# selftok-team/SelftokTokenizer

Hardware: NVIDIA H100
Metric: images/sec encode+50-step decode, 256x256/512-tok (higher is better)
Workload: dtype fp16 (IEEE-half operands on wgmma, fp32 accumulate; encoder/VQ/tables fp32)

## Files before the change

### selftoktokenizer_b200/csrc/gemm_tc.cu

```cuda
#include "common.cuh"
#include "hopper.cuh"
#include "kernels.h"

#include <stdlib.h>

namespace stk {

namespace {

using namespace hop;

constexpr int BM = 128, BN = 256, BK = 64, WK = 16;
constexpr int A_TILE_BYTES = BM * BK * 2;
constexpr int B_TILE_BYTES = BN * BK * 2;
constexpr int CONSUMERS = 2;
constexpr int NUM_THREADS = CONSUMERS * 128 + 128;
constexpr int PRODUCER_REGS = 40, CONSUMER_REGS = 232;
constexpr int ACC = BN / 2;
constexpr int kPrefetchKBlocks = 4;

template <int NSPLIT> struct Cfg {
  static constexpr int PLANES = NSPLIT == 3 ? 2 : 1;
  static constexpr int STAGE_BYTES = PLANES * (A_TILE_BYTES + B_TILE_BYTES);
  static constexpr int STAGES = NSPLIT == 3 ? 2 : 4;
  static constexpr int SMEM_BYTES = STAGES * STAGE_BYTES + 1024  + 256 ;
};

__device__ __forceinline__ void wgmma_tile(float (&d)[ACC], uint64_t da, uint64_t db, uint32_t acc, bool fp16) {
  if (fp16) wgmma_m64n256k16_ss_f16(d, da, db, acc);
  else wgmma_m64n256k16_ss_bf16(d, da, db, acc);
}

__device__ __forceinline__ float2 ldg2(const float* p) { return *reinterpret_cast<const float2*>(p); }

struct EpiRows {
  int orow[2], mrow[2];
  bool valid[2];
};

__device__ __forceinline__ EpiRows epilogue_rows(const Epilogue& e, int64_t row0, int64_t M) {
  const bool per_row_gate = e.mode == EPI_RESID && e.gate && (e.gate_period > 1 || e.tab_rows);
  const bool per_row_add = e.mode == EPI_STORE && e.addtab;
  EpiRows rw;
#pragma unroll
  for (int r = 0; r < 2; ++r) {
    const int64_t m = row0 + 8 * r;
    rw.valid[r] = m < M;
    const int mi = (int)m;
    rw.orow[r] = 0;
    if (e.row_map && rw.valid[r]) {
      rw.orow[r] = e.row_map[mi];
    } else if (e.plan && rw.valid[r]) {
      const int b = mi / e.rpb_in;
      const int n_img = e.rpb_out - (e.plan_ctx ? e.rpb_in : e.row_off);
      rw.orow[r] = b * e.rpb_out + plan_slot_row(mi % e.rpb_in, e.plan[2 * b], e.plan[2 * b + 1], n_img, e.plan_ctx != 0);
    } else if (rw.valid[r]) {
      rw.orow[r] = e.rpb_in > 0 ? (mi / e.rpb_in) * e.rpb_out + e.row_off + (mi % e.rpb_in) : mi;
    }
    if (e.tab_rows && rw.valid[r]) rw.mrow[r] = e.tab_rows[mi];
    else rw.mrow[r] = per_row_gate ? mi % e.gate_period : (per_row_add ? mi % e.add_period : 0);
  }
  return rw;
}

__device__ __forceinline__ void epilogue_prefetch(const Epilogue& e, const EpiRows& rw, int col0, int N) {
  if (e.mode != EPI_RESID) return;
  const int c0 = col0 & ~(BN - 1);
  const int q = (col0 >> 1) & 3;
#pragma unroll
  for (int r = 0; r < 2; ++r) {
#pragma unroll
    for (int h = 0; h < 2; ++h) {
      const int n = c0 + 32 * (2 * q + h);
      if (rw.valid[r] && n < N) prefetch_l2(e.resid + (int64_t)rw.orow[r] * e.ldo + n);
    }
  }
}

template <int MODE, bool GELU>
__device__ __forceinline__ void epilogue_tile(const Epilogue& e, const float (&acc)[ACC], const EpiRows& rw, int col0, int N) {
  constexpr int CH = MODE == EPI_RESID ? 4 : 8;
  const bool per_row_gate = MODE == EPI_RESID && e.gate && (e.gate_period > 1 || e.tab_rows);
  const bool per_row_add = MODE == EPI_STORE && e.addtab;
  const bool fp16 = e.fp16 != 0;
  const float2 zero = make_float2(0.f, 0.f), one = make_float2(1.f, 1.f);
#pragma unroll
  for (int c = 0; c < BN / 8; c += CH) {
    float2 bias[CH], res[2][CH], gt[2][CH], add[2][CH];
#pragma unroll
    for (int i = 0; i < CH; ++i) {
      const int n = col0 + 8 * (c + i);
      const bool in = n < N;
      bias[i] = e.bias && in ? ldg2(e.bias + n) : zero;
#pragma unroll
      for (int r = 0; r < 2; ++r) {
        const bool v = in && rw.valid[r];
        const int64_t o = (int64_t)rw.orow[r] * e.ldo + n;
        if (MODE == EPI_RESID) {
          res[r][i] = v ? ldg2(e.resid + o) : zero;
          gt[r][i] = v && e.gate ? ldg2(per_row_gate ? e.gate + (int64_t)rw.mrow[r] * e.gate_ld + n : e.gate + n) : one;
        }
        if (MODE == EPI_STORE) add[r][i] = v && per_row_add ? ldg2(e.addtab + (int64_t)rw.mrow[r] * e.add_ld + n) : zero;
      }
    }
#pragma unroll
    for (int i = 0; i < CH; ++i) {
      const int j = c + i;
      const int n = col0 + 8 * j;
      if (n >= N) continue;
#pragma unroll
      for (int r = 0; r < 2; ++r) {
        if (!rw.valid[r]) continue;
        float2 y = make_float2(acc[4 * j + 2 * r] + bias[i].x, acc[4 * j + 2 * r + 1] + bias[i].y);
        if (GELU) y = gelu_tanh_fast2(y);
        const int64_t o = (int64_t)rw.orow[r] * e.ldo + n;
        if (MODE == EPI_RESID) {
          y.x = fmaf(gt[r][i].x, y.x, res[r][i].x); y.y = fmaf(gt[r][i].y, y.y, res[r][i].y);
        }
        if (MODE == EPI_SPLIT) {
          const uint32_t hi = pack2_sat16(y.x, y.y, fp16);
          *reinterpret_cast<uint32_t*>(e.out_hi + o) = hi;
          if (e.out_lo) {
            const float lx = y.x - __bfloat162float(__float2bfloat16_rn(y.x)), ly = y.y - __bfloat162float(__float2bfloat16_rn(y.y));
            *reinterpret_cast<uint32_t*>(e.out_lo + o) = pack2_sat16(lx, ly, false);
          }
        } else {
          if (per_row_add) { y.x += add[r][i].x; y.y += add[r][i].y; }
          *reinterpret_cast<float2*>(e.out + o) = y;
        }
      }
    }
  }
}

__device__ __forceinline__ void epilogue_dispatch(const Epilogue& e, const float (&acc)[ACC], const EpiRows& rw, int col0, int N) {
  if (e.mode == EPI_RESID) epilogue_tile<EPI_RESID, false>(e, acc, rw, col0, N);
  else if (e.mode == EPI_SPLIT) {
    if (e.act == ACT_GELU) epilogue_tile<EPI_SPLIT, true>(e, acc, rw, col0, N);
    else epilogue_tile<EPI_SPLIT, false>(e, acc, rw, col0, N);
  } else {
    if (e.act == ACT_GELU) epilogue_tile<EPI_STORE, true>(e, acc, rw, col0, N);
    else epilogue_tile<EPI_STORE, false>(e, acc, rw, col0, N);
  }
}

struct TcMaps {
  CUtensorMap a_hi, a_lo, b_hi, b_lo;
};

struct GemmParams {
  int64_t M;
  int N, K;
  int fp16;
  Epilogue ep;
  int conv_C = 0, conv_H = 0, conv_W = 0, conv_stride = 1;
  int raster_gm = 4;
};

__device__ __forceinline__ void tile_coords(int t, int pm_tiles, int n_tiles, int GM, int& pm, int& n_blk) {
  const int per_group = GM * n_tiles;
  const int group = t / per_group;
  const int first = group * GM;
  const int gm = min(GM, pm_tiles - first);
  const int local = t - group * per_group;
  pm = first + local % gm;
  n_blk = local / gm;
}

template <int NSPLIT, int CL, bool FP16>
__global__ void __launch_bounds__(NUM_THREADS, 1)
gemm_tc_kernel(const __grid_constant__ TcMaps maps0, const __grid_constant__ TcMaps maps1, const GemmParams p0, const GemmParams p1) {
  static_assert(NSPLIT == 1 || !FP16, "the fp16 mode is single-pass");
  using C = Cfg<NSPLIT>;
  extern __shared__ uint8_t smem_raw[];
  const uint32_t smem_base = (smem_u32(smem_raw) + 1023u) & ~1023u;
  const uint32_t bar_base = smem_base + C::STAGES * C::STAGE_BYTES;
  auto full_bar = [&](int s) { return bar_base + 8u * s; };
  auto empty_bar = [&](int s) { return bar_base + 8u * (C::STAGES + s); };

  const int warp = threadIdx.x >> 5, lane = threadIdx.x & 31;
  const uint32_t rank = CL > 1 ? cluster_ctarank() : 0;
  const int pm_tiles0 = (int)((p0.M + CL * BM - 1) / (CL * BM)), n_tiles0 = (p0.N + BN - 1) / BN;
  const int pm_tiles1 = (int)((p1.M + CL * BM - 1) / (CL * BM)), n_tiles1 = (p1.N + BN - 1) / BN;
  const int tiles0 = pm_tiles0 * n_tiles0;
  const int num_tiles = tiles0 + pm_tiles1 * n_tiles1;
  const int cluster_id = blockIdx.x / CL, num_clusters = gridDim.x / CL;

  if (warp == CONSUMERS * 4 && lane == 0) {
    tma_prefetch_desc(&maps0.a_hi);
    tma_prefetch_desc(&maps0.b_hi);
    if (NSPLIT == 3) { tma_prefetch_desc(&maps0.a_lo); tma_prefetch_desc(&maps0.b_lo); }
    if (p1.M > 0) {
      tma_prefetch_desc(&maps1.a_hi);
      tma_prefetch_desc(&maps1.b_hi);
      if (NSPLIT == 3) { tma_prefetch_desc(&maps1.a_lo); tma_prefetch_desc(&maps1.b_lo); }
    }
    for (int s = 0; s < C::STAGES; ++s) { mbar_init(full_bar(s), 1); mbar_init(empty_bar(s), CONSUMERS * CL); }
    asm volatile("fence.mbarrier_init.release.cluster;" ::: "memory");
  }
  __syncthreads();
  if (CL > 1) cluster_sync_all();

  if (warp >= CONSUMERS * 4) {
    setmaxnreg_dec<PRODUCER_REGS>();
    if (warp == CONSUMERS * 4 && lane == 0) {
      int stage = 0; uint32_t phase = 0;
      const uint64_t w_policy = l2_policy_evict_last();
      for (int t = cluster_id; t < num_tiles; t += num_clusters) {
        const bool second = t >= tiles0;
        const TcMaps& mp = second ? maps1 : maps0;
        const GemmParams& pp = second ? p1 : p0;
        int pm, n_blk;
        if (second) tile_coords(t - tiles0, pm_tiles1, n_tiles1, p1.raster_gm, pm, n_blk);
        else tile_coords(t, pm_tiles0, n_tiles0, p0.raster_gm, pm, n_blk);
        const int nk = (pp.K + BK - 1) / BK;
        const int m_row = (pm * CL + (int)rank) * BM;
        const int n_row = n_blk * BN + (int)rank * (BN / CL);
        const int chunks = pp.conv_C > 0 ? pp.conv_C / BK : 1;
        int cx = 0, cy = 0, cb = 0;
        if (pp.conv_C > 0) {
          cx = m_row % pp.conv_W;
          cy = (m_row / pp.conv_W) % pp.conv_H;
          cb = m_row / (pp.conv_W * pp.conv_H);
        }
        for (int kb = 0; kb < nk; ++kb) {
          mbar_wait(empty_bar(stage), phase ^ 1);
          const uint32_t sa = smem_base + stage * C::STAGE_BYTES;
          const uint32_t sb = sa + C::PLANES * A_TILE_BYTES + (uint32_t)rank * (B_TILE_BYTES / CL);
          const uint32_t fb = full_bar(stage);
          mbar_expect_tx(fb, C::STAGE_BYTES);
          if (pp.conv_C > 0) {
            const int tap = kb / chunks, c0 = (kb - tap * chunks) * BK;
            const int dy = tap / 3, dx = tap - dy * 3;
            int x0 = cx + dx - 1, y0 = cy + dy - 1, n0 = cb;
            if (pp.conv_stride == 2) { x0 = cx + (dx >> 1); y0 = cy + (dy >> 1); n0 = cb * 4 + (dy & 1) * 2 + (dx & 1); }
            tma_load_4d(sa, &mp.a_hi, fb, c0, x0, y0, n0);
            if (NSPLIT == 3) tma_load_4d(sa + A_TILE_BYTES, &mp.a_lo, fb, c0, x0, y0, n0);
          } else {
            tma_load_2d(sa, &mp.a_hi, fb, kb * BK, m_row);
            if (NSPLIT == 3) tma_load_2d(sa + A_TILE_BYTES, &mp.a_lo, fb, kb * BK, m_row);
          }
          if (CL > 1) {
            tma_load_2d_mc(sb, &mp.b_hi, fb, kb * BK, n_row, (uint16_t)((1u << CL) - 1), w_policy);
            if (NSPLIT == 3) tma_load_2d_mc(sb + B_TILE_BYTES, &mp.b_lo, fb, kb * BK, n_row, (uint16_t)((1u << CL) - 1), w_policy);
          } else {
            tma_load_2d_hint(sb, &mp.b_hi, fb, kb * BK, n_row, w_policy);
            if (NSPLIT == 3) tma_load_2d_hint(sb + B_TILE_BYTES, &mp.b_lo, fb, kb * BK, n_row, w_policy);
          }
          if (++stage == C::STAGES) { stage = 0; phase ^= 1; }
        }
      }
    }
  } else {
    setmaxnreg_inc<CONSUMER_REGS>();
    const int wg = warp >> 2;
    const bool signaller = (threadIdx.x & 127) == 0;
    auto release = [&](int s) {
      if (!signaller) return;
      if (CL == 1) mbar_arrive(empty_bar(s));
      else for (int r = 0; r < CL; ++r) mbar_arrive_cluster(empty_bar(s), (uint32_t)r);
    };
    int stage = 0; uint32_t phase = 0;
    for (int t = cluster_id; t < num_tiles; t += num_clusters) {
      const bool second = t >= tiles0;
      int pm, n_blk;
      if (second) tile_coords(t - tiles0, pm_tiles1, n_tiles1, p1.raster_gm, pm, n_blk);
      else tile_coords(t, pm_tiles0, n_tiles0, p0.raster_gm, pm, n_blk);
      const int nk = ((second ? p1.K : p0.K) + BK - 1) / BK;
      const int wl = threadIdx.x & 127;
      const int64_t row0 = (int64_t)(pm * CL + (int)rank) * BM + wg * 64 + (wl >> 5) * 16 + ((wl & 31) >> 2);
      const int col0 = n_blk * BN + 2 * (wl & 3);
      const EpiRows rw = second ? epilogue_rows(p1.ep, row0, p1.M) : epilogue_rows(p0.ep, row0, p0.M);
      const int pf_kb = nk > kPrefetchKBlocks ? nk - kPrefetchKBlocks : 0;
      float acc[ACC];
#pragma unroll
      for (int i = 0; i < ACC; ++i) acc[i] = 0.f;
      int prev = -1;
      for (int kb = 0; kb < nk; ++kb) {
        mbar_wait(full_bar(stage), phase);
        const uint32_t sa_hi = smem_base + stage * C::STAGE_BYTES + wg * (64 * 128);
        const uint32_t sa_lo = sa_hi + A_TILE_BYTES;
        const uint32_t sb_hi = smem_base + stage * C::STAGE_BYTES + C::PLANES * A_TILE_BYTES;
        const uint32_t sb_lo = sb_hi + B_TILE_BYTES;
        wgmma_fence();
#pragma unroll
        for (int k = 0; k < BK / WK; ++k) {
          const uint32_t koff = k * WK * 2;
          const uint64_t da_hi = make_smem_desc(sa_hi + koff), db_hi = make_smem_desc(sb_hi + koff);
          wgmma_tile(acc, da_hi, db_hi, (kb > 0 || k > 0) ? 1u : 0u, FP16);
          if (NSPLIT == 3) {
            const uint64_t da_lo = make_smem_desc(sa_lo + koff), db_lo = make_smem_desc(sb_lo + koff);
            wgmma_tile(acc, da_hi, db_lo, 1u, false);
            wgmma_tile(acc, da_lo, db_hi, 1u, false);
          }
        }
        wgmma_commit();
        if (kb == pf_kb) {
          if (!second) epilogue_prefetch(p0.ep, rw, col0, p0.N);
          else epilogue_prefetch(p1.ep, rw, col0, p1.N);
        }
        wgmma_wait<1>();
        if (prev >= 0) release(prev);
        prev = stage;
        if (++stage == C::STAGES) { stage = 0; phase ^= 1; }
      }
      wgmma_wait<0>();
      fence_regs(acc);
      release(prev);
      if (!second) epilogue_dispatch(p0.ep, acc, rw, col0, p0.N);
      else epilogue_dispatch(p1.ep, acc, rw, col0, p1.N);
    }
  }
  if (CL > 1) cluster_sync_all();
}

typedef CUresult (*EncodeTiledFn)(CUtensorMap*, CUtensorMapDataType, cuuint32_t, void*, const cuuint64_t*, const cuuint64_t*,
                                  const cuuint32_t*, const cuuint32_t*, CUtensorMapInterleave, CUtensorMapSwizzle,
                                  CUtensorMapL2promotion, CUtensorMapFloatOOBfill);
EncodeTiledFn g_encode = nullptr;
constexpr int kMaxDev = 64;
int g_num_sms_dev[kMaxDev];
bool g_attr_dev[kMaxDev];
int g_raster_gm = 4;
int g_gemm_ctas = 2;

int make_map(CUtensorMap* map, const __nv_bfloat16* ptr, int64_t rows, int K, int box_rows, int fp16) {
  cuuint64_t gdim[2] = {(cuuint64_t)K, (cuuint64_t)rows};
  cuuint64_t gstride[1] = {(cuuint64_t)K * 2};
  cuuint32_t box[2] = {(cuuint32_t)BK, (cuuint32_t)box_rows};
  cuuint32_t estr[2] = {1, 1};
  CUresult r = g_encode(map, fp16 ? CU_TENSOR_MAP_DATA_TYPE_FLOAT16 : CU_TENSOR_MAP_DATA_TYPE_BFLOAT16, 2, const_cast<__nv_bfloat16*>(ptr), gdim, gstride, box, estr,
                        CU_TENSOR_MAP_INTERLEAVE_NONE, CU_TENSOR_MAP_SWIZZLE_128B, CU_TENSOR_MAP_L2_PROMOTION_L2_256B,
                        CU_TENSOR_MAP_FLOAT_OOB_FILL_NONE);
  if (r != CUDA_SUCCESS) {
    set_error("cuTensorMapEncodeTiled failed with CUresult " + std::to_string((int)r));
    return -5;
  }
  return 0;
}

int make_map_nhwc(CUtensorMap* map, const __nv_bfloat16* ptr, int64_t B, int H, int W, int Cc, int fp16) {
  const int bw = W < BM ? W : BM;
  const int bh = (BM / bw) < H ? (BM / bw) : H;
  const int bn = BM / (bw * bh);
  cuuint64_t gdim[4] = {(cuuint64_t)Cc, (cuuint64_t)W, (cuuint64_t)H, (cuuint64_t)B};
  cuuint64_t gstride[3] = {(cuuint64_t)Cc * 2, (cuuint64_t)W * Cc * 2, (cuuint64_t)H * W * Cc * 2};
  cuuint32_t box[4] = {(cuuint32_t)BK, (cuuint32_t)bw, (cuuint32_t)bh, (cuuint32_t)bn};
  cuuint32_t estr[4] = {1, 1, 1, 1};
  CUresult r = g_encode(map, fp16 ? CU_TENSOR_MAP_DATA_TYPE_FLOAT16 : CU_TENSOR_MAP_DATA_TYPE_BFLOAT16, 4, const_cast<__nv_bfloat16*>(ptr), gdim, gstride,
                        box, estr, CU_TENSOR_MAP_INTERLEAVE_NONE, CU_TENSOR_MAP_SWIZZLE_128B, CU_TENSOR_MAP_L2_PROMOTION_L2_256B,
                        CU_TENSOR_MAP_FLOAT_OOB_FILL_NONE);
  if (r != CUDA_SUCCESS) {
    set_error("cuTensorMapEncodeTiled (NHWC) failed with CUresult " + std::to_string((int)r));
    return -5;
  }
  return 0;
}

}

int make_tensor_map_2d(CUtensorMap* map, const void* ptr, uint64_t rows, uint64_t cols, uint32_t box_rows, uint32_t box_cols,
                       int fp16) {
  STK_CHECK(g_encode, -3, "gemm_tc_init has not been called");
  cuuint64_t gdim[2] = {(cuuint64_t)cols, (cuuint64_t)rows};
  cuuint64_t gstride[1] = {(cuuint64_t)cols * 2};
  cuuint32_t box[2] = {box_cols, box_rows};
  cuuint32_t estr[2] = {1, 1};
  CUresult r = g_encode(map, fp16 ? CU_TENSOR_MAP_DATA_TYPE_FLOAT16 : CU_TENSOR_MAP_DATA_TYPE_BFLOAT16, 2, const_cast<void*>(ptr), gdim,
                        gstride, box, estr, CU_TENSOR_MAP_INTERLEAVE_NONE, CU_TENSOR_MAP_SWIZZLE_128B,
                        CU_TENSOR_MAP_L2_PROMOTION_L2_256B, CU_TENSOR_MAP_FLOAT_OOB_FILL_NONE);
  if (r != CUDA_SUCCESS) {
    set_error("cuTensorMapEncodeTiled failed with CUresult " + std::to_string((int)r));
    return -5;
  }
  return 0;
}

void gemm_tc_set_ctas(int n) { g_gemm_ctas = n == 1 ? 1 : 2; }

int gemm_tc_init() {
  int dev = 0;
  STK_CUDA(cudaGetDevice(&dev));
  STK_CHECK(dev >= 0 && dev < kMaxDev, -1, "gemm_tc: device ordinal out of range");
  if (g_encode && g_attr_dev[dev]) return 0;
  if (!g_encode) {
    void* fn = nullptr;
    cudaDriverEntryPointQueryResult qres;
    STK_CUDA(cudaGetDriverEntryPoint("cuTensorMapEncodeTiled", &fn, cudaEnableDefault, &qres));
    STK_CHECK(fn && qres == cudaDriverEntryPointSuccess, -5, "cuTensorMapEncodeTiled not available from the driver");
    const char* v = getenv("SELFTOK_GEMM_CTAS");
    if (v) g_gemm_ctas = atoi(v) == 1 ? 1 : 2;
    const char* gm = getenv("SELFTOK_GEMM_GM");
    if (gm && atoi(gm) >= 1 && atoi(gm) <= 1024) g_raster_gm = atoi(gm);
    g_encode = reinterpret_cast<EncodeTiledFn>(fn);
  }
  STK_CUDA(cudaDeviceGetAttribute(&g_num_sms_dev[dev], cudaDevAttrMultiProcessorCount, dev));
  STK_CUDA(cudaFuncSetAttribute(gemm_tc_kernel<1, 1, false>, cudaFuncAttributeMaxDynamicSharedMemorySize, Cfg<1>::SMEM_BYTES));
  STK_CUDA(cudaFuncSetAttribute(gemm_tc_kernel<1, 1, true>, cudaFuncAttributeMaxDynamicSharedMemorySize, Cfg<1>::SMEM_BYTES));
  STK_CUDA(cudaFuncSetAttribute(gemm_tc_kernel<3, 1, false>, cudaFuncAttributeMaxDynamicSharedMemorySize, Cfg<3>::SMEM_BYTES));
  STK_CUDA(cudaFuncSetAttribute(gemm_tc_kernel<1, 2, false>, cudaFuncAttributeMaxDynamicSharedMemorySize, Cfg<1>::SMEM_BYTES));
  STK_CUDA(cudaFuncSetAttribute(gemm_tc_kernel<1, 2, true>, cudaFuncAttributeMaxDynamicSharedMemorySize, Cfg<1>::SMEM_BYTES));
  STK_CUDA(cudaFuncSetAttribute(gemm_tc_kernel<3, 2, false>, cudaFuncAttributeMaxDynamicSharedMemorySize, Cfg<3>::SMEM_BYTES));
  g_attr_dev[dev] = true;
  return 0;
}

int check_gemm_tc_problem(const TcProblem& q, int nsplit, int fp16) {
  const Epilogue& ep = q.ep;
  STK_CHECK(q.A_hi && q.W_hi && q.M > 0 && q.N > 0 && q.K > 0, -1, "gemm_tc: bad arguments");
  STK_CHECK(nsplit == 1 || (nsplit == 3 && q.A_lo && q.W_lo), -1, "gemm_tc: nsplit must be 1, or 3 with lo planes");
  STK_CHECK(!fp16 || nsplit == 1, -1, "gemm_tc: the fp16 mode is single-pass");
  auto aligned16 = [](const void* p) { return reinterpret_cast<uintptr_t>(p) % 16 == 0; };
  STK_CHECK(aligned16(q.A_hi) && aligned16(q.A_lo) && aligned16(q.W_hi) && aligned16(q.W_lo), -1,
            "gemm_tc: operand planes must be 16-byte aligned (TMA)");
  STK_TRY(check_epilogue(ep, "gemm_tc"));
  STK_CHECK(ep.act == ACT_NONE || (ep.act == ACT_GELU && ep.mode != EPI_RESID), -2,
            "gemm_tc: epilogue activation must be none, or GELU-tanh with the store / split modes");
  STK_CHECK(ep.mode != EPI_STORE || ep.addtab == nullptr || ep.add_ld % 4 == 0, -2, "gemm_tc: addtab pitch must be a multiple of 4");
  STK_CHECK(q.K % 8 == 0, -2, "gemm_tc: K must be a multiple of 8 (16-byte TMA row pitch)");
  STK_CHECK(ep.ldo % 4 == 0 && q.N % 4 == 0, -2, "gemm_tc: N and the output pitch must be multiples of 4");
  STK_CHECK(ep.mode != EPI_RESID || ep.gate == nullptr || ep.gate_ld % 4 == 0, -2, "gemm_tc: gate pitch must be a multiple of 4");
  if (q.conv_C > 0) {
    STK_CHECK(q.conv_C % BK == 0 && q.K == 9 * q.conv_C, -2, "gemm_tc conv: channels must be a multiple of 64 and K = 9 C");
    STK_CHECK(q.conv_W > 0 && q.conv_H > 0 && (q.conv_W % BM == 0 || BM % q.conv_W == 0), -2, "gemm_tc conv: image width must divide or be a multiple of 128");
    const int64_t hw = (int64_t)q.conv_H * q.conv_W;
    STK_CHECK(q.M % hw == 0 && (hw % BM == 0 || BM % hw == 0) && (q.conv_W >= BM || hw < BM || q.conv_H % (BM / q.conv_W) == 0), -2,
              "gemm_tc conv: 128-pixel tiles must be part of a row, whole rows of one image, or whole images");
    STK_CHECK(q.conv_stride == 1 || (q.conv_stride == 2 && hw % BM == 0), -2, "gemm_tc conv: stride 2 needs >= 128 output pixels per image");
  }
  return 0;
}

static int make_maps(TcMaps* m, const TcProblem& q, int nsplit, int fp16, int b_box) {
  const bool conv = q.conv_C > 0;
  const int64_t imgs = conv ? q.M / ((int64_t)q.conv_H * q.conv_W) * (q.conv_stride == 2 ? 4 : 1) : 0;
  if (conv) STK_TRY(make_map_nhwc(&m->a_hi, q.A_hi, imgs, q.conv_H, q.conv_W, q.conv_C, fp16));
  else STK_TRY(make_map(&m->a_hi, q.A_hi, q.M, q.K, BM, fp16));
  STK_TRY(make_map(&m->b_hi, q.W_hi, q.N, q.K, b_box, fp16));
  if (nsplit == 3) {
    if (conv) STK_TRY(make_map_nhwc(&m->a_lo, q.A_lo, imgs, q.conv_H, q.conv_W, q.conv_C, fp16));
    else STK_TRY(make_map(&m->a_lo, q.A_lo, q.M, q.K, BM, fp16));
    STK_TRY(make_map(&m->b_lo, q.W_lo, q.N, q.K, b_box, fp16));
  } else {
    m->a_lo = m->a_hi; m->b_lo = m->b_hi;
  }
  return 0;
}

template <int NSPLIT, int CL, bool FP16>
static int launch_kernel(const TcMaps& m0, const TcMaps& m1, const GemmParams& p0, const GemmParams& p1, int clusters, cudaStream_t s) {
  cudaLaunchConfig_t cfg = {};
  cfg.gridDim = dim3(CL * clusters);
  cfg.blockDim = dim3(NUM_THREADS);
  cfg.dynamicSmemBytes = Cfg<NSPLIT>::SMEM_BYTES;
  cfg.stream = s;
  cudaLaunchAttribute attr[1];
  attr[0].id = cudaLaunchAttributeClusterDimension;
  attr[0].val.clusterDim.x = CL; attr[0].val.clusterDim.y = 1; attr[0].val.clusterDim.z = 1;
  cfg.attrs = attr;
  cfg.numAttrs = 1;
  STK_CUDA(cudaLaunchKernelEx(&cfg, gemm_tc_kernel<NSPLIT, CL, FP16>, m0, m1, p0, p1));
  count_launch();
  return 0;
}

template <int CL>
static int launch_cl(const TcMaps& m0, const TcMaps& m1, const GemmParams& p0, const GemmParams& p1, int clusters, int nsplit, int fp16,
                     cudaStream_t s) {
  if (nsplit == 3) return launch_kernel<3, CL, false>(m0, m1, p0, p1, clusters, s);
  if (fp16) return launch_kernel<1, CL, true>(m0, m1, p0, p1, clusters, s);
  return launch_kernel<1, CL, false>(m0, m1, p0, p1, clusters, s);
}

int launch_gemm_tc_grouped(const TcProblem* probs, int n, int nsplit, cudaStream_t s, int fp16) {
  STK_TRY(gemm_tc_init());
  STK_CHECK(probs && (n == 1 || n == 2), -1, "gemm_tc: one or two problems per launch");
  int dev = 0;
  STK_CUDA(cudaGetDevice(&dev));
  const int g_num_sms = g_num_sms_dev[dev];
  for (int i = 0; i < n; ++i) STK_TRY(check_gemm_tc_problem(probs[i], nsplit, fp16));
  const int CL = g_gemm_ctas == 2 && g_num_sms >= 2 ? 2 : 1;
  TcMaps m0, m1;
  STK_TRY(make_maps(&m0, probs[0], nsplit, fp16, BN / CL));
  auto mk_params = [&](const TcProblem& q) {
    GemmParams g{q.M, q.N, q.K, fp16, q.ep};
    g.conv_C = q.conv_C; g.conv_H = q.conv_H; g.conv_W = q.conv_W; g.conv_stride = q.conv_stride;
    g.raster_gm = g_raster_gm;
    return g;
  };
  GemmParams p0 = mk_params(probs[0]);
  GemmParams p1 = p0;
  p1.M = 0;
  m1 = m0;
  int tiles = (int)((probs[0].M + CL * BM - 1) / (CL * BM)) * ((probs[0].N + BN - 1) / BN);
  if (n == 2) {
    STK_TRY(make_maps(&m1, probs[1], nsplit, fp16, BN / CL));
    p1 = mk_params(probs[1]);
    tiles += (int)((probs[1].M + CL * BM - 1) / (CL * BM)) * ((probs[1].N + BN - 1) / BN);
  }
  const int clusters = tiles < g_num_sms / CL ? tiles : g_num_sms / CL;
  if (CL == 2) return launch_cl<2>(m0, m1, p0, p1, clusters, nsplit, fp16, s);
  return launch_cl<1>(m0, m1, p0, p1, clusters, nsplit, fp16, s);
}

int launch_gemm_tc(const __nv_bfloat16* A_hi, const __nv_bfloat16* A_lo, const __nv_bfloat16* W_hi,
                   const __nv_bfloat16* W_lo, int64_t M, int N, int K, int nsplit, const Epilogue& ep,
                   cudaStream_t s, int fp16) {
  TcProblem q{A_hi, A_lo, W_hi, W_lo, M, N, K, ep};
  return launch_gemm_tc_grouped(&q, 1, nsplit, s, fp16);
}

}
```

### selftoktokenizer_b200/csrc/hopper.cuh

```cuda
#pragma once
#include <cuda.h>
#include <stdint.h>

namespace stk {
namespace hop {

__device__ __forceinline__ uint32_t smem_u32(const void* p) { return (uint32_t)__cvta_generic_to_shared(p); }

__device__ __forceinline__ void mbar_init(uint32_t bar, uint32_t count) {
  asm volatile("mbarrier.init.shared::cta.b64 [%0], %1;" ::"r"(bar), "r"(count) : "memory");
}
__device__ __forceinline__ void mbar_expect_tx(uint32_t bar, uint32_t bytes) {
  asm volatile("mbarrier.arrive.expect_tx.shared::cta.b64 _, [%0], %1;" ::"r"(bar), "r"(bytes) : "memory");
}
__device__ __forceinline__ void mbar_arrive(uint32_t bar) {
  asm volatile("mbarrier.arrive.shared::cta.b64 _, [%0];" ::"r"(bar) : "memory");
}
__device__ __forceinline__ void mbar_arrive_cluster(uint32_t local_bar, uint32_t rank) {
  asm volatile(
      "{\n\t.reg .b32 ra;\n\t"
      "mapa.shared::cluster.u32 ra, %0, %1;\n\t"
      "mbarrier.arrive.shared::cluster.b64 _, [ra];\n\t}"
      ::"r"(local_bar), "r"(rank) : "memory");
}
constexpr uint32_t kSuspendHintNs = 20000;
__device__ __forceinline__ bool mbar_try_wait(uint32_t bar, uint32_t parity) {
  uint32_t ok;
  asm volatile(
      "{\n\t.reg .pred p;\n\t"
      "mbarrier.try_wait.parity.shared::cta.b64 p, [%1], %2, %3;\n\t"
      "selp.u32 %0, 1, 0, p;\n\t}"
      : "=r"(ok) : "r"(bar), "r"(parity), "r"(kSuspendHintNs) : "memory");
  return ok != 0;
}
__device__ __forceinline__ void mbar_wait(uint32_t bar, uint32_t parity) {
  if (mbar_try_wait(bar, parity)) return;
  const long long t0 = clock64();
  uint32_t spins = 0;
  while (!mbar_try_wait(bar, parity)) {
    if ((++spins & 0x3ff) == 0 && clock64() - t0 > 8000000000LL) __trap();
  }
}

__device__ __forceinline__ void tma_prefetch_desc(const CUtensorMap* map) {
  asm volatile("prefetch.tensormap [%0];" ::"l"(reinterpret_cast<uint64_t>(map)) : "memory");
}
__device__ __forceinline__ void tma_load_2d(uint32_t dst, const CUtensorMap* map, uint32_t bar, int c0, int c1) {
  asm volatile(
      "cp.async.bulk.tensor.2d.shared::cluster.global.mbarrier::complete_tx::bytes [%0], [%1, {%3, %4}], [%2];"
      ::"r"(dst), "l"(reinterpret_cast<uint64_t>(map)), "r"(bar), "r"(c0), "r"(c1) : "memory");
}
__device__ __forceinline__ void tma_load_4d(uint32_t dst, const CUtensorMap* map, uint32_t bar, int c0, int c1, int c2, int c3) {
  asm volatile(
      "cp.async.bulk.tensor.4d.shared::cluster.global.mbarrier::complete_tx::bytes [%0], [%1, {%3, %4, %5, %6}], [%2];"
      ::"r"(dst), "l"(reinterpret_cast<uint64_t>(map)), "r"(bar), "r"(c0), "r"(c1), "r"(c2), "r"(c3) : "memory");
}
__device__ __forceinline__ void tma_load_2d_mc(uint32_t dst, const CUtensorMap* map, uint32_t bar, int c0, int c1, uint16_t mask,
                                               uint64_t policy) {
  asm volatile(
      "cp.async.bulk.tensor.2d.shared::cluster.global.mbarrier::complete_tx::bytes.multicast::cluster.L2::cache_hint"
      " [%0], [%1, {%3, %4}], [%2], %5, %6;"
      ::"r"(dst), "l"(reinterpret_cast<uint64_t>(map)), "r"(bar), "r"(c0), "r"(c1), "h"(mask), "l"(policy) : "memory");
}
__device__ __forceinline__ void tma_load_2d_hint(uint32_t dst, const CUtensorMap* map, uint32_t bar, int c0, int c1, uint64_t policy) {
  asm volatile(
      "cp.async.bulk.tensor.2d.shared::cluster.global.mbarrier::complete_tx::bytes.L2::cache_hint [%0], [%1, {%3, %4}], [%2], %5;"
      ::"r"(dst), "l"(reinterpret_cast<uint64_t>(map)), "r"(bar), "r"(c0), "r"(c1), "l"(policy) : "memory");
}
__device__ __forceinline__ uint64_t l2_policy_evict_last() {
  uint64_t pol;
  asm volatile("createpolicy.fractional.L2::evict_last.b64 %0, 1.0;" : "=l"(pol));
  return pol;
}

template <int R> __device__ __forceinline__ void setmaxnreg_inc() { asm volatile("setmaxnreg.inc.sync.aligned.u32 %0;" ::"n"(R)); }
template <int R> __device__ __forceinline__ void setmaxnreg_dec() { asm volatile("setmaxnreg.dec.sync.aligned.u32 %0;" ::"n"(R)); }

__device__ __forceinline__ void prefetch_l2(const void* p) {
  asm volatile("prefetch.global.L2 [%0];" ::"l"(reinterpret_cast<uint64_t>(p)));
}

__device__ __forceinline__ uint32_t cluster_ctarank() {
  uint32_t r;
  asm volatile("mov.u32 %0, %%cluster_ctarank;" : "=r"(r));
  return r;
}
__device__ __forceinline__ void cluster_sync_all() {
  asm volatile("barrier.cluster.arrive.release.aligned;\n\tbarrier.cluster.wait.acquire.aligned;" ::: "memory");
}

__device__ __forceinline__ uint64_t make_smem_desc(uint32_t smem_addr) {
  uint64_t d = 0;
  d |= (uint64_t)((smem_addr >> 4) & 0x3FFF);
  d |= (uint64_t)1 << 16;
  d |= (uint64_t)(1024 >> 4) << 32;
  d |= (uint64_t)1 << 62;
  return d;
}
__device__ __forceinline__ void wgmma_fence() { asm volatile("wgmma.fence.sync.aligned;" ::: "memory"); }
__device__ __forceinline__ void wgmma_commit() { asm volatile("wgmma.commit_group.sync.aligned;" ::: "memory"); }
template <int N>
__device__ __forceinline__ void wgmma_wait() { asm volatile("wgmma.wait_group.sync.aligned %0;" ::"n"(N) : "memory"); }
template <int R>
__device__ __forceinline__ void fence_regs(float (&d)[R]) {
#pragma unroll
  for (int i = 0; i < R; ++i) asm volatile("" : "+f"(d[i])::"memory");
}

#define STK_WGMMA_SS_N256(NAME, T)                                                                                   \
  __device__ __forceinline__ void NAME(float (&d)[128], uint64_t da, uint64_t db, uint32_t accumulate) { \
    asm volatile("{\n\t.reg .pred p;\n\tsetp.ne.b32 p, %130, 0;\n\t"                                             \
                 "wgmma.mma_async.sync.aligned.m64n256k16.f32." T "." T " "                                             \
                 "{%0, %1, %2, %3, %4, %5, %6, %7, %8, %9, %10, %11, %12, %13, %14, %15, %16, %17, %18, %19, %20, %21, %22, %23, %24, %25, %26, %27, %28, %29, %30, %31, %32, %33, %34, %35, %36, %37, %38, %39, %40, %41, %42, %43, %44, %45, %46, %47, %48, %49, %50, %51, %52, %53, %54, %55, %56, %57, %58, %59, %60, %61, %62, %63, %64, %65, %66, %67, %68, %69, %70, %71, %72, %73, %74, %75, %76, %77, %78, %79, %80, %81, %82, %83, %84, %85, %86, %87, %88, %89, %90, %91, %92, %93, %94, %95, %96, %97, %98, %99, %100, %101, %102, %103, %104, %105, %106, %107, %108, %109, %110, %111, %112, %113, %114, %115, %116, %117, %118, %119, %120, %121, %122, %123, %124, %125, %126, %127}, "  \
                 "%128, %129, p, 1, 1, 0, 0;\n\t}"                                                                  \
                 : "+f"(d[0]), "+f"(d[1]), "+f"(d[2]), "+f"(d[3]), "+f"(d[4]), "+f"(d[5]), "+f"(d[6]), "+f"(d[7]), "+f"(d[8]), "+f"(d[9]), "+f"(d[10]), "+f"(d[11]), "+f"(d[12]), "+f"(d[13]), "+f"(d[14]), "+f"(d[15]), "+f"(d[16]), "+f"(d[17]), "+f"(d[18]), "+f"(d[19]), "+f"(d[20]), "+f"(d[21]), "+f"(d[22]), "+f"(d[23]), "+f"(d[24]), "+f"(d[25]), "+f"(d[26]), "+f"(d[27]), "+f"(d[28]), "+f"(d[29]), "+f"(d[30]), "+f"(d[31]), "+f"(d[32]), "+f"(d[33]), "+f"(d[34]), "+f"(d[35]), "+f"(d[36]), "+f"(d[37]), "+f"(d[38]), "+f"(d[39]), "+f"(d[40]), "+f"(d[41]), "+f"(d[42]), "+f"(d[43]), "+f"(d[44]), "+f"(d[45]), "+f"(d[46]), "+f"(d[47]), "+f"(d[48]), "+f"(d[49]), "+f"(d[50]), "+f"(d[51]), "+f"(d[52]), "+f"(d[53]), "+f"(d[54]), "+f"(d[55]), "+f"(d[56]), "+f"(d[57]), "+f"(d[58]), "+f"(d[59]), "+f"(d[60]), "+f"(d[61]), "+f"(d[62]), "+f"(d[63]), "+f"(d[64]), "+f"(d[65]), "+f"(d[66]), "+f"(d[67]), "+f"(d[68]), "+f"(d[69]), "+f"(d[70]), "+f"(d[71]), "+f"(d[72]), "+f"(d[73]), "+f"(d[74]), "+f"(d[75]), "+f"(d[76]), "+f"(d[77]), "+f"(d[78]), "+f"(d[79]), "+f"(d[80]), "+f"(d[81]), "+f"(d[82]), "+f"(d[83]), "+f"(d[84]), "+f"(d[85]), "+f"(d[86]), "+f"(d[87]), "+f"(d[88]), "+f"(d[89]), "+f"(d[90]), "+f"(d[91]), "+f"(d[92]), "+f"(d[93]), "+f"(d[94]), "+f"(d[95]), "+f"(d[96]), "+f"(d[97]), "+f"(d[98]), "+f"(d[99]), "+f"(d[100]), "+f"(d[101]), "+f"(d[102]), "+f"(d[103]), "+f"(d[104]), "+f"(d[105]), "+f"(d[106]), "+f"(d[107]), "+f"(d[108]), "+f"(d[109]), "+f"(d[110]), "+f"(d[111]), "+f"(d[112]), "+f"(d[113]), "+f"(d[114]), "+f"(d[115]), "+f"(d[116]), "+f"(d[117]), "+f"(d[118]), "+f"(d[119]), "+f"(d[120]), "+f"(d[121]), "+f"(d[122]), "+f"(d[123]), "+f"(d[124]), "+f"(d[125]), "+f"(d[126]), "+f"(d[127]) \
                 : "l"(da), "l"(db), "r"(accumulate));                                                                         \
  }
STK_WGMMA_SS_N256(wgmma_m64n256k16_ss_bf16, "bf16")
STK_WGMMA_SS_N256(wgmma_m64n256k16_ss_f16, "f16")

#define STK_WGMMA_SS_N64(NAME, T)                                                                                   \
  __device__ __forceinline__ void NAME(float (&d)[32], uint64_t da, uint64_t db, uint32_t accumulate) { \
    asm volatile("{\n\t.reg .pred p;\n\tsetp.ne.b32 p, %34, 0;\n\t"                                             \
                 "wgmma.mma_async.sync.aligned.m64n64k16.f32." T "." T " "                                             \
                 "{%0, %1, %2, %3, %4, %5, %6, %7, %8, %9, %10, %11, %12, %13, %14, %15, %16, %17, %18, %19, %20, %21, %22, %23, %24, %25, %26, %27, %28, %29, %30, %31}, "  \
                 "%32, %33, p, 1, 1, 0, 0;\n\t}"                                                                  \
                 : "+f"(d[0]), "+f"(d[1]), "+f"(d[2]), "+f"(d[3]), "+f"(d[4]), "+f"(d[5]), "+f"(d[6]), "+f"(d[7]), "+f"(d[8]), "+f"(d[9]), "+f"(d[10]), "+f"(d[11]), "+f"(d[12]), "+f"(d[13]), "+f"(d[14]), "+f"(d[15]), "+f"(d[16]), "+f"(d[17]), "+f"(d[18]), "+f"(d[19]), "+f"(d[20]), "+f"(d[21]), "+f"(d[22]), "+f"(d[23]), "+f"(d[24]), "+f"(d[25]), "+f"(d[26]), "+f"(d[27]), "+f"(d[28]), "+f"(d[29]), "+f"(d[30]), "+f"(d[31]) \
                 : "l"(da), "l"(db), "r"(accumulate));                                                                         \
  }
STK_WGMMA_SS_N64(wgmma_m64n64k16_ss_bf16, "bf16")
STK_WGMMA_SS_N64(wgmma_m64n64k16_ss_f16, "f16")

#define STK_WGMMA_RS_N64(NAME, T)                                                                                   \
  __device__ __forceinline__ void NAME(float (&d)[32], const uint32_t (&a)[4], uint64_t db, uint32_t accumulate) { \
    asm volatile("{\n\t.reg .pred p;\n\tsetp.ne.b32 p, %37, 0;\n\t"                                             \
                 "wgmma.mma_async.sync.aligned.m64n64k16.f32." T "." T " "                                             \
                 "{%0, %1, %2, %3, %4, %5, %6, %7, %8, %9, %10, %11, %12, %13, %14, %15, %16, %17, %18, %19, %20, %21, %22, %23, %24, %25, %26, %27, %28, %29, %30, %31}, "  \
                 "{%32, %33, %34, %35}, %36, p, 1, 1, 1;\n\t}"                                                                  \
                 : "+f"(d[0]), "+f"(d[1]), "+f"(d[2]), "+f"(d[3]), "+f"(d[4]), "+f"(d[5]), "+f"(d[6]), "+f"(d[7]), "+f"(d[8]), "+f"(d[9]), "+f"(d[10]), "+f"(d[11]), "+f"(d[12]), "+f"(d[13]), "+f"(d[14]), "+f"(d[15]), "+f"(d[16]), "+f"(d[17]), "+f"(d[18]), "+f"(d[19]), "+f"(d[20]), "+f"(d[21]), "+f"(d[22]), "+f"(d[23]), "+f"(d[24]), "+f"(d[25]), "+f"(d[26]), "+f"(d[27]), "+f"(d[28]), "+f"(d[29]), "+f"(d[30]), "+f"(d[31]) \
                 : "r"(a[0]), "r"(a[1]), "r"(a[2]), "r"(a[3]), "l"(db), "r"(accumulate));                                                                         \
  }
STK_WGMMA_RS_N64(wgmma_m64n64k16_rs_bf16, "bf16")
STK_WGMMA_RS_N64(wgmma_m64n64k16_rs_f16, "f16")

}
}
```

Before: 9.959.

## Add ping-pong consumer schedule with 64-row tiles for short-K GEMMs

Adds a ping-pong variant of the warp-specialized GEMM, used when the problem is single-pass, not a convolution, and has K up to 1536. In this variant each consumer warpgroup owns alternate 64x256 tiles, and named barriers order their mainloops so one group's epilogue overlaps the other group's MMA. The A tile shrinks to 64 rows and there are 5 pipeline stages. This targets the exposed epilogue cost on short-K GEMMs, which dominate the decoder, at the price of twice as many tiles and more reloads of B per output row. The skip logic that advances the stage and phase has to stay in exact step with the producer.

```diff
diff --git a/selftoktokenizer_b200/csrc/gemm_tc.cu b/selftoktokenizer_b200/csrc/gemm_tc.cu
--- a/selftoktokenizer_b200/csrc/gemm_tc.cu
+++ b/selftoktokenizer_b200/csrc/gemm_tc.cu
@@ -11,18 +11,21 @@
 using namespace hop;
 
 constexpr int BM = 128, BN = 256, BK = 64, WK = 16;
-constexpr int A_TILE_BYTES = BM * BK * 2;
 constexpr int B_TILE_BYTES = BN * BK * 2;
 constexpr int CONSUMERS = 2;
+constexpr int kPingPongMaxK = 1536;
+constexpr int kMainloopBar = 1;
 constexpr int NUM_THREADS = CONSUMERS * 128 + 128;
 constexpr int PRODUCER_REGS = 40, CONSUMER_REGS = 232;
 constexpr int ACC = BN / 2;
 constexpr int kPrefetchKBlocks = 4;
 
-template <int NSPLIT> struct Cfg {
+template <int NSPLIT, bool PP> struct Cfg {
   static constexpr int PLANES = NSPLIT == 3 ? 2 : 1;
+  static constexpr int TM = PP ? 64 : BM;
+  static constexpr int A_TILE_BYTES = TM * BK * 2;
   static constexpr int STAGE_BYTES = PLANES * (A_TILE_BYTES + B_TILE_BYTES);
-  static constexpr int STAGES = NSPLIT == 3 ? 2 : 4;
+  static constexpr int STAGES = NSPLIT == 3 ? 2 : PP ? 5 : 4;
   static constexpr int SMEM_BYTES = STAGES * STAGE_BYTES + 1024  + 256 ;
 };
 
@@ -167,11 +170,11 @@
   n_blk = local / gm;
 }
 
-template <int NSPLIT, int CL, bool FP16>
+template <int NSPLIT, int CL, bool FP16, bool PP>
 __global__ void __launch_bounds__(NUM_THREADS, 1)
 gemm_tc_kernel(const __grid_constant__ TcMaps maps0, const __grid_constant__ TcMaps maps1, const GemmParams p0, const GemmParams p1) {
   static_assert(NSPLIT == 1 || !FP16, "the fp16 mode is single-pass");
-  using C = Cfg<NSPLIT>;
+  using C = Cfg<NSPLIT, PP>;
   extern __shared__ uint8_t smem_raw[];
   const uint32_t smem_base = (smem_u32(smem_raw) + 1023u) & ~1023u;
   const uint32_t bar_base = smem_base + C::STAGES * C::STAGE_BYTES;
@@ -180,8 +183,8 @@
 
   const int warp = threadIdx.x >> 5, lane = threadIdx.x & 31;
   const uint32_t rank = CL > 1 ? cluster_ctarank() : 0;
-  const int pm_tiles0 = (int)((p0.M + CL * BM - 1) / (CL * BM)), n_tiles0 = (p0.N + BN - 1) / BN;
-  const int pm_tiles1 = (int)((p1.M + CL * BM - 1) / (CL * BM)), n_tiles1 = (p1.N + BN - 1) / BN;
+  const int pm_tiles0 = (int)((p0.M + CL * C::TM - 1) / (CL * C::TM)), n_tiles0 = (p0.N + BN - 1) / BN;
+  const int pm_tiles1 = (int)((p1.M + CL * C::TM - 1) / (CL * C::TM)), n_tiles1 = (p1.N + BN - 1) / BN;
   const int tiles0 = pm_tiles0 * n_tiles0;
   const int num_tiles = tiles0 + pm_tiles1 * n_tiles1;
   const int cluster_id = blockIdx.x / CL, num_clusters = gridDim.x / CL;
@@ -195,7 +198,7 @@
       tma_prefetch_desc(&maps1.b_hi);
       if (NSPLIT == 3) { tma_prefetch_desc(&maps1.a_lo); tma_prefetch_desc(&maps1.b_lo); }
     }
-    for (int s = 0; s < C::STAGES; ++s) { mbar_init(full_bar(s), 1); mbar_init(empty_bar(s), CONSUMERS * CL); }
+    for (int s = 0; s < C::STAGES; ++s) { mbar_init(full_bar(s), 1); mbar_init(empty_bar(s), (PP ? 1 : CONSUMERS) * CL); }
     asm volatile("fence.mbarrier_init.release.cluster;" ::: "memory");
   }
   __syncthreads();
@@ -214,7 +217,7 @@
         if (second) tile_coords(t - tiles0, pm_tiles1, n_tiles1, p1.raster_gm, pm, n_blk);
         else tile_coords(t, pm_tiles0, n_tiles0, p0.raster_gm, pm, n_blk);
         const int nk = (pp.K + BK - 1) / BK;
-        const int m_row = (pm * CL + (int)rank) * BM;
+        const int m_row = (pm * CL + (int)rank) * C::TM;
         const int n_row = n_blk * BN + (int)rank * (BN / CL);
         const int chunks = pp.conv_C > 0 ? pp.conv_C / BK : 1;
         int cx = 0, cy = 0, cb = 0;
@@ -226,7 +229,7 @@
         for (int kb = 0; kb < nk; ++kb) {
           mbar_wait(empty_bar(stage), phase ^ 1);
           const uint32_t sa = smem_base + stage * C::STAGE_BYTES;
-          const uint32_t sb = sa + C::PLANES * A_TILE_BYTES + (uint32_t)rank * (B_TILE_BYTES / CL);
+          const uint32_t sb = sa + C::PLANES * C::A_TILE_BYTES + (uint32_t)rank * (B_TILE_BYTES / CL);
           const uint32_t fb = full_bar(stage);
           mbar_expect_tx(fb, C::STAGE_BYTES);
           if (pp.conv_C > 0) {
@@ -235,10 +238,10 @@
             int x0 = cx + dx - 1, y0 = cy + dy - 1, n0 = cb;
             if (pp.conv_stride == 2) { x0 = cx + (dx >> 1); y0 = cy + (dy >> 1); n0 = cb * 4 + (dy & 1) * 2 + (dx & 1); }
             tma_load_4d(sa, &mp.a_hi, fb, c0, x0, y0, n0);
-            if (NSPLIT == 3) tma_load_4d(sa + A_TILE_BYTES, &mp.a_lo, fb, c0, x0, y0, n0);
+            if (NSPLIT == 3) tma_load_4d(sa + C::A_TILE_BYTES, &mp.a_lo, fb, c0, x0, y0, n0);
           } else {
             tma_load_2d(sa, &mp.a_hi, fb, kb * BK, m_row);
-            if (NSPLIT == 3) tma_load_2d(sa + A_TILE_BYTES, &mp.a_lo, fb, kb * BK, m_row);
+            if (NSPLIT == 3) tma_load_2d(sa + C::A_TILE_BYTES, &mp.a_lo, fb, kb * BK, m_row);
           }
           if (CL > 1) {
             tma_load_2d_mc(sb, &mp.b_hi, fb, kb * BK, n_row, (uint16_t)((1u << CL) - 1), w_policy);
@@ -261,26 +264,35 @@
       else for (int r = 0; r < CL; ++r) mbar_arrive_cluster(empty_bar(s), (uint32_t)r);
     };
     int stage = 0; uint32_t phase = 0;
-    for (int t = cluster_id; t < num_tiles; t += num_clusters) {
+    int it = 0;
+    for (int t = cluster_id; t < num_tiles; t += num_clusters, ++it) {
       const bool second = t >= tiles0;
+      const int nk = ((second ? p1.K : p0.K) + BK - 1) / BK;
+      if (PP && (it & 1) != wg) {
+        stage += nk;
+        phase ^= (uint32_t)(stage / C::STAGES) & 1u;
+        stage %= C::STAGES;
+        continue;
+      }
       int pm, n_blk;
       if (second) tile_coords(t - tiles0, pm_tiles1, n_tiles1, p1.raster_gm, pm, n_blk);
       else tile_coords(t, pm_tiles0, n_tiles0, p0.raster_gm, pm, n_blk);
-      const int nk = ((second ? p1.K : p0.K) + BK - 1) / BK;
       const int wl = threadIdx.x & 127;
-      const int64_t row0 = (int64_t)(pm * CL + (int)rank) * BM + wg * 64 + (wl >> 5) * 16 + ((wl & 31) >> 2);
+      const int wrow = PP ? 0 : wg * 64;
+      const int64_t row0 = (int64_t)(pm * CL + (int)rank) * C::TM + wrow + (wl >> 5) * 16 + ((wl & 31) >> 2);
       const int col0 = n_blk * BN + 2 * (wl & 3);
       const EpiRows rw = second ? epilogue_rows(p1.ep, row0, p1.M) : epilogue_rows(p0.ep, row0, p0.M);
       const int pf_kb = nk > kPrefetchKBlocks ? nk - kPrefetchKBlocks : 0;
       float acc[ACC];
 #pragma unroll
       for (int i = 0; i < ACC; ++i) acc[i] = 0.f;
+      if (PP && it > 0) bar_sync(kMainloopBar + wg, CONSUMERS * 128);
       int prev = -1;
       for (int kb = 0; kb < nk; ++kb) {
         mbar_wait(full_bar(stage), phase);
-        const uint32_t sa_hi = smem_base + stage * C::STAGE_BYTES + wg * (64 * 128);
-        const uint32_t sa_lo = sa_hi + A_TILE_BYTES;
-        const uint32_t sb_hi = smem_base + stage * C::STAGE_BYTES + C::PLANES * A_TILE_BYTES;
+        const uint32_t sa_hi = smem_base + stage * C::STAGE_BYTES + wrow * 128;
+        const uint32_t sa_lo = sa_hi + C::A_TILE_BYTES;
+        const uint32_t sb_hi = smem_base + stage * C::STAGE_BYTES + C::PLANES * C::A_TILE_BYTES;
         const uint32_t sb_lo = sb_hi + B_TILE_BYTES;
         wgmma_fence();
 #pragma unroll
@@ -304,6 +316,7 @@
         prev = stage;
         if (++stage == C::STAGES) { stage = 0; phase ^= 1; }
       }
+      if (PP && t + num_clusters < num_tiles) bar_arrive(kMainloopBar + (wg ^ 1), CONSUMERS * 128);
       wgmma_wait<0>();
       fence_regs(acc);
       release(prev);
@@ -377,6 +390,15 @@
 }
 
 void gemm_tc_set_ctas(int n) { g_gemm_ctas = n == 1 ? 1 : 2; }
+
+template <int CL, bool PP>
+static int set_smem_attr() {
+  STK_CUDA(cudaFuncSetAttribute(gemm_tc_kernel<1, CL, false, PP>, cudaFuncAttributeMaxDynamicSharedMemorySize, Cfg<1, PP>::SMEM_BYTES));
+  STK_CUDA(cudaFuncSetAttribute(gemm_tc_kernel<1, CL, true, PP>, cudaFuncAttributeMaxDynamicSharedMemorySize, Cfg<1, PP>::SMEM_BYTES));
+  if (!PP)
+    STK_CUDA(cudaFuncSetAttribute(gemm_tc_kernel<3, CL, false, false>, cudaFuncAttributeMaxDynamicSharedMemorySize, Cfg<3, false>::SMEM_BYTES));
+  return 0;
+}
 
 int gemm_tc_init() {
   int dev = 0;
@@ -395,12 +417,10 @@
     g_encode = reinterpret_cast<EncodeTiledFn>(fn);
   }
   STK_CUDA(cudaDeviceGetAttribute(&g_num_sms_dev[dev], cudaDevAttrMultiProcessorCount, dev));
-  STK_CUDA(cudaFuncSetAttribute(gemm_tc_kernel<1, 1, false>, cudaFuncAttributeMaxDynamicSharedMemorySize, Cfg<1>::SMEM_BYTES));
-  STK_CUDA(cudaFuncSetAttribute(gemm_tc_kernel<1, 1, true>, cudaFuncAttributeMaxDynamicSharedMemorySize, Cfg<1>::SMEM_BYTES));
-  STK_CUDA(cudaFuncSetAttribute(gemm_tc_kernel<3, 1, false>, cudaFuncAttributeMaxDynamicSharedMemorySize, Cfg<3>::SMEM_BYTES));
-  STK_CUDA(cudaFuncSetAttribute(gemm_tc_kernel<1, 2, false>, cudaFuncAttributeMaxDynamicSharedMemorySize, Cfg<1>::SMEM_BYTES));
-  STK_CUDA(cudaFuncSetAttribute(gemm_tc_kernel<1, 2, true>, cudaFuncAttributeMaxDynamicSharedMemorySize, Cfg<1>::SMEM_BYTES));
-  STK_CUDA(cudaFuncSetAttribute(gemm_tc_kernel<3, 2, false>, cudaFuncAttributeMaxDynamicSharedMemorySize, Cfg<3>::SMEM_BYTES));
+  STK_TRY((set_smem_attr<1, false>()));
+  STK_TRY((set_smem_attr<2, false>()));
+  STK_TRY((set_smem_attr<1, true>()));
+  STK_TRY((set_smem_attr<2, true>()));
   g_attr_dev[dev] = true;
   return 0;
 }
@@ -431,15 +451,15 @@
   return 0;
 }
 
-static int make_maps(TcMaps* m, const TcProblem& q, int nsplit, int fp16, int b_box) {
+static int make_maps(TcMaps* m, const TcProblem& q, int nsplit, int fp16, int a_box, int b_box) {
   const bool conv = q.conv_C > 0;
   const int64_t imgs = conv ? q.M / ((int64_t)q.conv_H * q.conv_W) * (q.conv_stride == 2 ? 4 : 1) : 0;
   if (conv) STK_TRY(make_map_nhwc(&m->a_hi, q.A_hi, imgs, q.conv_H, q.conv_W, q.conv_C, fp16));
-  else STK_TRY(make_map(&m->a_hi, q.A_hi, q.M, q.K, BM, fp16));
+  else STK_TRY(make_map(&m->a_hi, q.A_hi, q.M, q.K, a_box, fp16));
   STK_TRY(make_map(&m->b_hi, q.W_hi, q.N, q.K, b_box, fp16));
   if (nsplit == 3) {
     if (conv) STK_TRY(make_map_nhwc(&m->a_lo, q.A_lo, imgs, q.conv_H, q.conv_W, q.conv_C, fp16));
-    else STK_TRY(make_map(&m->a_lo, q.A_lo, q.M, q.K, BM, fp16));
+    else STK_TRY(make_map(&m->a_lo, q.A_lo, q.M, q.K, a_box, fp16));
     STK_TRY(make_map(&m->b_lo, q.W_lo, q.N, q.K, b_box, fp16));
   } else {
     m->a_lo = m->a_hi; m->b_lo = m->b_hi;
@@ -447,29 +467,30 @@
   return 0;
 }
 
-template <int NSPLIT, int CL, bool FP16>
+template <int NSPLIT, int CL, bool FP16, bool PP>
 static int launch_kernel(const TcMaps& m0, const TcMaps& m1, const GemmParams& p0, const GemmParams& p1, int clusters, cudaStream_t s) {
   cudaLaunchConfig_t cfg = {};
   cfg.gridDim = dim3(CL * clusters);
   cfg.blockDim = dim3(NUM_THREADS);
-  cfg.dynamicSmemBytes = Cfg<NSPLIT>::SMEM_BYTES;
+  cfg.dynamicSmemBytes = Cfg<NSPLIT, PP>::SMEM_BYTES;
   cfg.stream = s;
   cudaLaunchAttribute attr[1];
   attr[0].id = cudaLaunchAttributeClusterDimension;
   attr[0].val.clusterDim.x = CL; attr[0].val.clusterDim.y = 1; attr[0].val.clusterDim.z = 1;
   cfg.attrs = attr;
   cfg.numAttrs = 1;
-  STK_CUDA(cudaLaunchKernelEx(&cfg, gemm_tc_kernel<NSPLIT, CL, FP16>, m0, m1, p0, p1));
+  STK_CUDA(cudaLaunchKernelEx(&cfg, gemm_tc_kernel<NSPLIT, CL, FP16, PP>, m0, m1, p0, p1));
   count_launch();
   return 0;
 }
 
 template <int CL>
 static int launch_cl(const TcMaps& m0, const TcMaps& m1, const GemmParams& p0, const GemmParams& p1, int clusters, int nsplit, int fp16,
-                     cudaStream_t s) {
-  if (nsplit == 3) return launch_kernel<3, CL, false>(m0, m1, p0, p1, clusters, s);
-  if (fp16) return launch_kernel<1, CL, true>(m0, m1, p0, p1, clusters, s);
-  return launch_kernel<1, CL, false>(m0, m1, p0, p1, clusters, s);
+                     bool pp, cudaStream_t s) {
+  if (nsplit == 3) return launch_kernel<3, CL, false, false>(m0, m1, p0, p1, clusters, s);
+  if (pp) return fp16 ? launch_kernel<1, CL, true, true>(m0, m1, p0, p1, clusters, s) : launch_kernel<1, CL, false, true>(m0, m1, p0, p1, clusters, s);
+  if (fp16) return launch_kernel<1, CL, true, false>(m0, m1, p0, p1, clusters, s);
+  return launch_kernel<1, CL, false, false>(m0, m1, p0, p1, clusters, s);
 }
 
 int launch_gemm_tc_grouped(const TcProblem* probs, int n, int nsplit, cudaStream_t s, int fp16) {
@@ -480,8 +501,11 @@
   const int g_num_sms = g_num_sms_dev[dev];
   for (int i = 0; i < n; ++i) STK_TRY(check_gemm_tc_problem(probs[i], nsplit, fp16));
   const int CL = g_gemm_ctas == 2 && g_num_sms >= 2 ? 2 : 1;
+  bool pp = nsplit == 1;
+  for (int i = 0; i < n; ++i) pp = pp && probs[i].conv_C == 0 && probs[i].K <= kPingPongMaxK;
+  const int TM = pp ? Cfg<1, true>::TM : BM;
   TcMaps m0, m1;
-  STK_TRY(make_maps(&m0, probs[0], nsplit, fp16, BN / CL));
+  STK_TRY(make_maps(&m0, probs[0], nsplit, fp16, TM, BN / CL));
   auto mk_params = [&](const TcProblem& q) {
     GemmParams g{q.M, q.N, q.K, fp16, q.ep};
     g.conv_C = q.conv_C; g.conv_H = q.conv_H; g.conv_W = q.conv_W; g.conv_stride = q.conv_stride;
@@ -492,15 +516,15 @@
   GemmParams p1 = p0;
   p1.M = 0;
   m1 = m0;
-  int tiles = (int)((probs[0].M + CL * BM - 1) / (CL * BM)) * ((probs[0].N + BN - 1) / BN);
+  int tiles = (int)((probs[0].M + CL * TM - 1) / (CL * TM)) * ((probs[0].N + BN - 1) / BN);
   if (n == 2) {
-    STK_TRY(make_maps(&m1, probs[1], nsplit, fp16, BN / CL));
+    STK_TRY(make_maps(&m1, probs[1], nsplit, fp16, TM, BN / CL));
     p1 = mk_params(probs[1]);
-    tiles += (int)((probs[1].M + CL * BM - 1) / (CL * BM)) * ((probs[1].N + BN - 1) / BN);
+    tiles += (int)((probs[1].M + CL * TM - 1) / (CL * TM)) * ((probs[1].N + BN - 1) / BN);
   }
   const int clusters = tiles < g_num_sms / CL ? tiles : g_num_sms / CL;
-  if (CL == 2) return launch_cl<2>(m0, m1, p0, p1, clusters, nsplit, fp16, s);
-  return launch_cl<1>(m0, m1, p0, p1, clusters, nsplit, fp16, s);
+  if (CL == 2) return launch_cl<2>(m0, m1, p0, p1, clusters, nsplit, fp16, pp, s);
+  return launch_cl<1>(m0, m1, p0, p1, clusters, nsplit, fp16, pp, s);
 }
 
 int launch_gemm_tc(const __nv_bfloat16* A_hi, const __nv_bfloat16* A_lo, const __nv_bfloat16* W_hi,
diff --git a/selftoktokenizer_b200/csrc/hopper.cuh b/selftoktokenizer_b200/csrc/hopper.cuh
--- a/selftoktokenizer_b200/csrc/hopper.cuh
+++ b/selftoktokenizer_b200/csrc/hopper.cuh
@@ -80,6 +80,13 @@
   asm volatile("prefetch.global.L2 [%0];" ::"l"(reinterpret_cast<uint64_t>(p)));
 }
 
+__device__ __forceinline__ void bar_sync(int id, int threads) {
+  asm volatile("bar.sync %0, %1;" ::"r"(id), "r"(threads) : "memory");
+}
+__device__ __forceinline__ void bar_arrive(int id, int threads) {
+  asm volatile("bar.arrive %0, %1;" ::"r"(id), "r"(threads) : "memory");
+}
+
 __device__ __forceinline__ uint32_t cluster_ctarank() {
   uint32_t r;
   asm volatile("mov.u32 %0, %%cluster_ctarank;" : "=r"(r));
```

After: 10.09, median of 6. 1.01x the previous value.
